# ronghanghu/vit_10b_fsdp_example

Measured on AMD Instinct MI355X. Metric: images/sec (whole node) for ViT-10B bs=128 224px --fake_data, higher is better.
Workload: dtype bf16; 1 GPU; model=ViT-10B (5120d/32h/32L, patch14, 224px), global_batch=128, seq_len=256, parallelism=fsdp1, grad_ckpt=True, grad_ckpt_blocks=13, fuse_residual=False, init=device

## Files before the change

__graft_entry__.py:

```python

import os
import subprocess
import sys


def build():
    env = dict(os.environ)
    env["PYTORCH_ROCM_ARCH"] = "gfx950"
    env.setdefault("MAX_JOBS", "8")
    repo = os.path.dirname(os.path.abspath(__file__))
    subprocess.check_call(
        [sys.executable, "setup.py", "build_ext", "--inplace"],
        cwd=repo, env=env,
    )
    import torch
    import vit_10b_fsdp_example_amd
    import vit_10b_fsdp_example_amd._C as _C

    required = [
        "layernorm_fwd", "layernorm_bwd", "layernorm_add_fwd",
        "fused_adamw", "multi_tensor_sqnorm", "cross_entropy_fwd",
        "fmha_fwd", "fmha_bwd", "fmha_fwd_qkv", "wgrad_gemm", "lt_gemm",
        "fwd_gemm", "fwd_gemm_gelu", "mfma32_probe",
    ]
    missing = [f for f in required if not hasattr(_C, f)]
    assert not missing, f"extension missing symbols: {missing}"
    print("build OK: vit_10b_fsdp_example_amd._C (gfx950)")


def smoke():
    import torch

    assert torch.cuda.is_available(), "smoke() needs a GPU"
    from vit_10b_fsdp_example_amd import dist as xdist
    from vit_10b_fsdp_example_amd.cli import parse_args
    from vit_10b_fsdp_example_amd.models import build_fsdp_vit_model
    from vit_10b_fsdp_example_amd.ops import (
        CrossEntropyLoss, FusedAdamW, has_ext,
    )

    assert has_ext(), "HIP extension _C not importable on the GPU box"
    device = xdist.init_distributed()
    cfg = parse_args([
        "--fake_data", "--image_size", "224", "--patch_size", "14",
        "--embed_dim", "640", "--num_heads", "4", "--num_blocks", "2",
        "--num_classes", "1000", "--batch_size", "8", "--num_workers", "0",
# ... 23 lines not shown
```

csrc/bindings.cpp:

```cpp

#include <torch/extension.h>

std::vector<torch::Tensor> layernorm_fwd(torch::Tensor x, torch::Tensor w,
                                         torch::Tensor b, double eps);
std::vector<torch::Tensor> layernorm_bwd(torch::Tensor dy, torch::Tensor x,
                                         torch::Tensor w, torch::Tensor mean,
                                         torch::Tensor rstd);
std::vector<torch::Tensor> layernorm_add_fwd(torch::Tensor x,
                                             torch::Tensor res,
                                             torch::Tensor w, torch::Tensor b,
                                             double eps);
std::vector<torch::Tensor> layernorm_add_bwd(torch::Tensor dy,
                                             torch::Tensor dsum,
                                             torch::Tensor sum,
                                             torch::Tensor w,
                                             torch::Tensor mean,
                                             torch::Tensor rstd);

void fused_adamw(std::vector<torch::Tensor> params,
                 std::vector<torch::Tensor> grads,
                 std::vector<torch::Tensor> exp_avgs,
                 std::vector<torch::Tensor> exp_avg_sqs,
                 std::vector<c10::optional<torch::Tensor>> mirrors,
                 double lr,
// ... 5 lines not shown
void multi_tensor_scale(std::vector<torch::Tensor> tensors, double factor);
void multi_tensor_scale_tensor(std::vector<torch::Tensor> tensors,
                               torch::Tensor factor);

std::vector<torch::Tensor> cross_entropy_fwd(torch::Tensor logits,
                                             torch::Tensor target);
torch::Tensor cross_entropy_bwd(torch::Tensor dloss, torch::Tensor logits,
                                torch::Tensor target, torch::Tensor lse);

std::vector<torch::Tensor> fmha_fwd(torch::Tensor q, torch::Tensor k,
                                    torch::Tensor v, double scale,
                                    double p_drop, long seed);
std::vector<torch::Tensor> fmha_bwd(torch::Tensor dout, torch::Tensor q,
                                    torch::Tensor k, torch::Tensor v,
                                    torch::Tensor o, torch::Tensor lse,
                                    double scale, double p_drop, long seed);
std::vector<torch::Tensor> fmha_fwd_qkv(torch::Tensor qkv, long num_heads,
                                        double scale, double p_drop,
                                        long seed);
torch::Tensor fmha_bwd_qkv(torch::Tensor dout, torch::Tensor qkv,
                           torch::Tensor o, torch::Tensor lse,
                           long num_heads, double scale, double p_drop,
                           long seed);
torch::Tensor mfma_probe(torch::Tensor a, torch::Tensor b);
torch::Tensor mfma32_probe(torch::Tensor a, torch::Tensor b);
torch::Tensor tr16_probe(long mode);
std::vector<torch::Tensor> wgrad_gemm(torch::Tensor a, torch::Tensor b,
                                      bool with_bias);
torch::Tensor fwd_gemm(torch::Tensor x, torch::Tensor w,
                       c10::optional<torch::Tensor> bias);
std::vector<torch::Tensor> fwd_gemm_gelu(torch::Tensor x, torch::Tensor w,
                                         torch::Tensor bias);
torch::Tensor lt_gemm(torch::Tensor a, torch::Tensor b, long algo_index,
                      c10::optional<torch::Tensor> bias);
std::vector<torch::Tensor> lt_gemm_gelu(torch::Tensor a, torch::Tensor b,
                                        c10::optional<torch::Tensor> bias,
                                        long algo_index);
std::vector<torch::Tensor> lt_gemm_dgelu_bgrad(torch::Tensor dy,
                                               torch::Tensor w,
                                               torch::Tensor aux,
                                               long algo_index);

PYBIND11_MODULE(TORCH_EXTENSION_NAME, m) {
  m.doc() = "MI355X-native CDNA4 kernels for the FSDP ViT framework";
  m.def("layernorm_fwd", &layernorm_fwd, "LayerNorm forward (bf16, fp32 stats)");
  m.def("layernorm_bwd", &layernorm_bwd, "LayerNorm backward");
// ... 17 lines not shown
  m.def("cross_entropy_fwd", &cross_entropy_fwd, "fused softmax CE forward");
  m.def("cross_entropy_bwd", &cross_entropy_bwd, "fused softmax CE backward");
  m.def("fmha_fwd", &fmha_fwd,
        "flash attention forward (bf16, head_dim<=192; in-kernel "
        "attention dropout via a counter-hash mask)",
        py::arg("q"), py::arg("k"), py::arg("v"), py::arg("scale"),
        py::arg("p_drop") = 0.0, py::arg("seed") = 0);
  m.def("fmha_bwd", &fmha_bwd,
        "flash attention backward (fused FA2-style; regenerates the "
        "dropout mask from the seed)",
        py::arg("dout"), py::arg("q"), py::arg("k"), py::arg("v"),
        py::arg("o"), py::arg("lse"), py::arg("scale"),
        py::arg("p_drop") = 0.0, py::arg("seed") = 0);
  m.def("fmha_fwd_qkv", &fmha_fwd_qkv,
        "flash attention forward on the fused [B,T,3,H,D] qkv projection "
        "(zero-copy strided IO, O returned as [B,T,E])",
        py::arg("qkv"), py::arg("num_heads"), py::arg("scale"),
        py::arg("p_drop") = 0.0, py::arg("seed") = 0);
  m.def("fmha_bwd_qkv", &fmha_bwd_qkv,
        "flash attention backward producing the fused dqkv [B,T,3,H,D]",
        py::arg("dout"), py::arg("qkv"), py::arg("o"), py::arg("lse"),
        py::arg("num_heads"), py::arg("scale"), py::arg("p_drop") = 0.0,
        py::arg("seed") = 0);
  m.def("mfma_probe", &mfma_probe, "16x16x32 bf16 MFMA layout probe");
  m.def("mfma32_probe", &mfma32_probe, "32x32x16 bf16 MFMA layout probe");
  m.def("tr16_probe", &tr16_probe, "ds_read_b64_tr_b16 semantics probe");
  m.def("wgrad_gemm", &wgrad_gemm,
        "C = A^T B weight-gradient GEMM (bf16, tr16 transpose reads)");
  m.def("fwd_gemm", &fwd_gemm,
        "C = X W^T forward Linear GEMM (+fused bias), hand-written CDNA4 "
        "MFMA (csrc/fgemm.hip)",
        py::arg("x"), py::arg("w"), py::arg("bias") = py::none());
  m.def("fwd_gemm_gelu", &fwd_gemm_gelu,
        "(gelu(X W^T + bias), pre-activation) with the EXACT erf GELU "
        "fused into the hand-written forward GEMM epilogue",
        py::arg("x"), py::arg("w"), py::arg("bias"));
  m.def("lt_gemm", &lt_gemm,
        "row-major bf16 GEMM (+optional fused bias epilogue) via "
        "hipblaslt-ext with an explicit algorithm index (-1 = library "
        "heuristic); offline-search apply path, see "
        "csrc/tools/hipblaslt_search.cpp",
        py::arg("a"), py::arg("b"), py::arg("algo_index") = -1,
        py::arg("bias") = py::none());
  m.def("lt_gemm_gelu", &lt_gemm_gelu,
        "(gelu(a@b+bias), pre-activation aux) in one hipblaslt-ext GEMM "
        "(GELU_AUX epilogue; tanh-approx GELU)",
// ... 9 lines not shown
```

csrc/fmha.hip:

```cpp

#ifndef VITFSDP_KERNELS_ONLY
#include <ATen/cuda/CUDAContext.h>
#include <torch/extension.h>

#include <cstdlib>
#include <cstring>
#include <type_traits>
#endif

#include "mfma_tiles.h"

namespace {

constexpr int kBlockThreads = 256;
constexpr int kKTile = 32;
constexpr int kMaxD = 192;

template <int D>
struct FmhaShapes {
  static constexpr int QSub = (D <= 96) ? 2 : 1;
  static constexpr int QTile = 64 * QSub;
  static constexpr int DP = ((D + 31) / 32) * 32;
  static constexpr int NKC = DP / 32;
  static constexpr int NC = D / 16;
// ... 488 lines not shown
        base0 + (unsigned)offsetof(typename S::SharedDKV, do_tile);
    mfma_tr_ring<NC, S::KStride>(pt_frag, do_lds_base, seg, col, dv_acc);
    mfma_tr_ring<NC, S::KStride>(dst_frag, q_lds_base, seg, col, dk_acc);
    if (has_next) {
      __syncthreads();
      write_qdo_tiles();
      __syncthreads();
    }
  }

#pragma unroll
  for (int r = 0; r < 4; ++r) {
    const int k_row = k_row0 + seg * 4 + r;
    if (k_row >= T) continue;
    const long out_base = qkv_off + (long)k_row * st.qt;
#pragma unroll
    for (int c = 0; c < NC; ++c) {
      dk[out_base + c * 16 + col] = (short)f32_to_bf16(dk_acc[c][r]);
      dv[out_base + c * 16 + col] = (short)f32_to_bf16(dv_acc[c][r]);
    }
  }
}

__global__ __launch_bounds__(64) void fmha_rowdot_kernel(
    const unsigned short* __restrict__ dout,
    const unsigned short* __restrict__ o, float* __restrict__ delta, int T,
    int H, int D, long sob, long soh, long sot) {
  const long row = blockIdx.x;
  const int t = (int)(row % T);
  const int h = (int)((row / T) % H);
  const long b = row / ((long)T * H);
  const long base = b * sob + (long)h * soh + (long)t * sot;
  float acc = 0.f;
  for (int i = threadIdx.x; i < D; i += 64)
    acc += bf16_to_f32(dout[base + i]) * bf16_to_f32(o[base + i]);
  acc = wave_all_sum(acc);
  if (threadIdx.x == 0) delta[row] = acc;
}

__global__ __launch_bounds__(256) void fmha_dsoftmax_kernel(
    const unsigned short* __restrict__ s_raw,
    const unsigned short* __restrict__ dp, const float* __restrict__ lse,
    const float* __restrict__ delta, unsigned short* __restrict__ p_out,
    unsigned short* __restrict__ ds_out, int T, float scale) {
  const long row = blockIdx.x;
  const float row_lse = lse[row];
  const float row_delta = delta[row];
// ... 146 lines not shown
  st.qb = (long)H * st.qh;
  st.qt = D;
  st.ob = st.qb;
  st.oh = st.qh;
  st.ot = st.qt;
  return st;
}

QkvStrides fused_qkv_strides(int T, int H, int D) {
  QkvStrides st;
  st.qt = 3L * H * D;
  st.qb = (long)T * st.qt;
  st.qh = D;
  st.ot = (long)H * D;
  st.ob = (long)T * st.ot;
  st.oh = D;
  return st;
}

torch::Tensor run_rowdot(const torch::Tensor& dout, const torch::Tensor& o,
                         int B, int H, int T, int D, const QkvStrides& st) {
  auto delta = torch::empty({B, H, T}, dout.options().dtype(torch::kFloat32));
  auto stream = at::cuda::getCurrentCUDAStream();
  hipLaunchKernelGGL(fmha_rowdot_kernel, dim3((long)B * H * T), dim3(64), 0,
                     stream, (const unsigned short*)dout.data_ptr(),
                     (const unsigned short*)o.data_ptr(),
                     delta.data_ptr<float>(), T, H, D, st.ob, st.oh, st.ot);
  HIP_CHECK_LAST();
  return delta;
}

}


std::vector<torch::Tensor> fmha_fwd(torch::Tensor q, torch::Tensor k,
                                    torch::Tensor v, double scale,
                                    double p_drop, long seed) {
  TORCH_CHECK(q.is_cuda() && q.is_contiguous() && k.is_contiguous() &&
              v.is_contiguous());
  TORCH_CHECK(q.scalar_type() == torch::kBFloat16, "fmha_fwd: bf16 only");
  TORCH_CHECK(q.dim() == 4, "fmha_fwd: [B, H, T, D]");
  const int B = q.size(0), H = q.size(1), T = q.size(2), D = q.size(3);
  TORCH_CHECK(D % 16 == 0 && D <= kMaxD,
              "fmha_fwd: head_dim must be a multiple of 16 and <= ", kMaxD);

  auto o = torch::empty_like(q);
  auto lse = torch::empty({B, H, T}, q.options().dtype(torch::kFloat32));
  FmhaArgs a{(const short*)q.data_ptr(), (const short*)k.data_ptr(),
             (const short*)v.data_ptr(), (short*)o.data_ptr(),
             B, H, T, contiguous_strides(H, T, D), (float)scale,
// ... 26 lines not shown
                       (const unsigned short*)dp.data_ptr(),
                       lse.data_ptr<float>(), delta.data_ptr<float>(),
                       (unsigned short*)p.data_ptr(),
                       (unsigned short*)ds.data_ptr(), T, (float)scale);
    HIP_CHECK_LAST();
    auto dv = at::matmul(p.transpose(-2, -1), dout);
    auto dq = at::matmul(ds, k);
    auto dk = at::matmul(ds.transpose(-2, -1), q);
    return {dq, dk, dv};
  }

  auto dq = torch::empty_like(q);
  auto dk = torch::empty_like(k);
  auto dv = torch::empty_like(v);
  FmhaArgs a{(const short*)q.data_ptr(), (const short*)k.data_ptr(),
             (const short*)v.data_ptr(), (short*)dout.data_ptr(),
             B, H, T, st, (float)scale, (float)p_drop, (unsigned)seed};
  VITFSDP_FMHA_DISPATCH(
      D, launch_fmha_bwd<kD>(a, lse, delta, (short*)dq.data_ptr(),
                             (short*)dk.data_ptr(), (short*)dv.data_ptr()));
  return {dq, dk, dv};
}


std::vector<torch::Tensor> fmha_fwd_qkv(torch::Tensor qkv, long num_heads,
                                        double scale, double p_drop,
                                        long seed) {
  TORCH_CHECK(qkv.is_cuda() && qkv.is_contiguous() && qkv.dim() == 5 &&
                  qkv.size(2) == 3 && qkv.size(3) == num_heads,
              "fmha_fwd_qkv: expected contiguous [B, T, 3, H, D]");
  TORCH_CHECK(qkv.scalar_type() == torch::kBFloat16, "fmha: bf16 only");
  const int B = qkv.size(0), T = qkv.size(1), H = qkv.size(3),
            D = qkv.size(4);
  TORCH_CHECK(D % 16 == 0 && D <= kMaxD,
              "fmha: head_dim must be a multiple of 16 and <= ", kMaxD);
  const QkvStrides st = fused_qkv_strides(T, H, D);

  auto o = torch::empty({B, T, (long)H * D}, qkv.options());
  auto lse = torch::empty({B, H, T}, qkv.options().dtype(torch::kFloat32));
  const short* base = (const short*)qkv.data_ptr();
  FmhaArgs a{base, base + (long)H * D, base + 2L * H * D,
             (short*)o.data_ptr(), B, H, T, st, (float)scale,
             (float)p_drop, (unsigned)seed};
  VITFSDP_FMHA_DISPATCH(D, launch_fmha_fwd<kD>(a, lse));
  return {o, lse};
}
// ... 24 lines not shown
```

csrc/layernorm.hip:

```cpp

#ifndef VITFSDP_KERNELS_ONLY
#include <ATen/cuda/CUDAContext.h>
#include <torch/extension.h>
#endif

#include "common.h"

namespace {

constexpr int kBlock = 256;
constexpr int kWaves = kBlock / WAVE_SIZE;

__global__ void ln_fwd_kernel(const ushort8_t* __restrict__ x,
                              const ushort8_t* __restrict__ w,
                              const ushort8_t* __restrict__ b,
                              ushort8_t* __restrict__ y,
                              float* __restrict__ mean_out,
                              float* __restrict__ rstd_out, int nvec,
                              float inv_d, float eps) {
  __shared__ float scratch[kWaves];
  const long row = blockIdx.x;
  const ushort8_t* xr = x + row * nvec;
  ushort8_t* yr = y + row * nvec;

// ... 69 lines not shown
  }
}

__global__ void ln_bwd_dwdb_partial_kernel(
    const unsigned short* __restrict__ dy, const unsigned short* __restrict__ x,
    const float* __restrict__ mean_in, const float* __restrict__ rstd_in,
    float* __restrict__ dw_part, float* __restrict__ db_part, int d,
    long n_rows, int rows_per_chunk) {
  const int col = blockIdx.x * kBlock + threadIdx.x;
  if (col >= d) return;
  const long row_begin = (long)blockIdx.y * rows_per_chunk;
  const long row_end = min(row_begin + rows_per_chunk, n_rows);
  float dw = 0.f, db = 0.f;
  for (long r = row_begin; r < row_end; ++r) {
    float dyv = bf16_to_f32(dy[r * d + col]);
    float xh = (bf16_to_f32(x[r * d + col]) - mean_in[r]) * rstd_in[r];
    dw += dyv * xh;
    db += dyv;
  }
  dw_part[(long)blockIdx.y * d + col] = dw;
  db_part[(long)blockIdx.y * d + col] = db;
}

__global__ void ln_bwd_dwdb_final_kernel(const float* __restrict__ dw_part,
                                         const float* __restrict__ db_part,
                                         unsigned short* __restrict__ dw,
                                         unsigned short* __restrict__ db,
                                         int d, int n_chunks) {
  const int col = blockIdx.x * kBlock + threadIdx.x;
  if (col >= d) return;
  float sw = 0.f, sb = 0.f;
  for (int c = 0; c < n_chunks; ++c) {
    sw += dw_part[(long)c * d + col];
    sb += db_part[(long)c * d + col];
  }
  dw[col] = f32_to_bf16(sw);
  db[col] = f32_to_bf16(sb);
}


__global__ void ln_add_fwd_kernel(const ushort8_t* __restrict__ x,
                                  const ushort8_t* __restrict__ res,
                                  const ushort8_t* __restrict__ w,
                                  const ushort8_t* __restrict__ b,
                                  ushort8_t* __restrict__ sum_out,
                                  ushort8_t* __restrict__ y,
                                  float* __restrict__ mean_out,
                                  float* __restrict__ rstd_out, int nvec,
                                  float inv_d, float eps) {
  __shared__ float scratch[kWaves];
  const long row = blockIdx.x;
  const ushort8_t* xr = x + row * nvec;
  const ushort8_t* rr = res + row * nvec;
  ushort8_t* sr = sum_out + row * nvec;
  ushort8_t* yr = y + row * nvec;

  float s = 0.f, ss = 0.f;
  for (int i = threadIdx.x; i < nvec; i += kBlock) {
    ushort8_t xv = xr[i], rv = rr[i], sv;
#pragma unroll
    for (int j = 0; j < 8; ++j) {
// ... 55 lines not shown
      sg += g;
      sgx += g * xh;
    }
  }
  sg = block_sum<kWaves>(sg, scratch) * inv_d;
  sgx = block_sum<kWaves>(sgx, scratch) * inv_d;

  for (int i = threadIdx.x; i < nvec; i += kBlock) {
    ushort8_t dv = dyr[i], sv = sr[i], wv = w[i], av = dsr[i], out;
#pragma unroll
    for (int j = 0; j < 8; ++j) {
      float g = bf16_to_f32(dv[j]) * bf16_to_f32(wv[j]);
      float xh = (bf16_to_f32(sv[j]) - mean) * rstd;
      out[j] = f32_to_bf16(rstd * (g - sg - xh * sgx) + bf16_to_f32(av[j]));
    }
    d1[i] = out;
    d2[i] = out;
  }
}

}

#ifndef VITFSDP_KERNELS_ONLY
std::vector<torch::Tensor> layernorm_fwd(torch::Tensor x, torch::Tensor w,
                                         torch::Tensor b, double eps) {
  TORCH_CHECK(x.is_cuda() && x.is_contiguous());
  TORCH_CHECK(x.scalar_type() == torch::kBFloat16, "layernorm_fwd: bf16 only");
  const int d = x.size(-1);
  TORCH_CHECK(d % 8 == 0, "layernorm_fwd: D must be a multiple of 8");
  const long n = x.numel() / d;
  auto y = torch::empty_like(x);
  auto opts = x.options().dtype(torch::kFloat32);
  auto mean = torch::empty({n}, opts);
  auto rstd = torch::empty({n}, opts);
  auto stream = at::cuda::getCurrentCUDAStream();
  hipLaunchKernelGGL(ln_fwd_kernel, dim3((unsigned)n), dim3(kBlock), 0, stream,
                     (const ushort8_t*)x.data_ptr(),
                     (const ushort8_t*)w.data_ptr(),
                     (const ushort8_t*)b.data_ptr(), (ushort8_t*)y.data_ptr(),
                     mean.data_ptr<float>(), rstd.data_ptr<float>(), d / 8,
                     1.f / d, (float)eps);
  HIP_CHECK_LAST();
  return {y, mean, rstd};
}

std::vector<torch::Tensor> layernorm_bwd(torch::Tensor dy, torch::Tensor x,
                                         torch::Tensor w, torch::Tensor mean,
                                         torch::Tensor rstd) {
  TORCH_CHECK(dy.is_cuda() && dy.is_contiguous() && x.is_contiguous());
  const int d = x.size(-1);
  const long n = x.numel() / d;
  auto dx = torch::empty_like(x);
  auto dw = torch::empty_like(w);
  auto db = torch::empty_like(w);
  auto stream = at::cuda::getCurrentCUDAStream();
  hipLaunchKernelGGL(ln_bwd_dx_kernel, dim3((unsigned)n), dim3(kBlock), 0,
                     stream, (const ushort8_t*)dy.data_ptr(),
                     (const ushort8_t*)x.data_ptr(),
                     (const ushort8_t*)w.data_ptr(), mean.data_ptr<float>(),
                     rstd.data_ptr<float>(), (ushort8_t*)dx.data_ptr(), d / 8,
                     1.f / d);
  HIP_CHECK_LAST();

  const int grid_x = (d + kBlock - 1) / kBlock;
  int n_chunks = std::max(1, 2048 / std::max(grid_x, 1));
  int rows_per_chunk = (int)((n + n_chunks - 1) / n_chunks);
  rows_per_chunk = std::max(rows_per_chunk, 16);
  n_chunks = (int)((n + rows_per_chunk - 1) / rows_per_chunk);
  auto opts = x.options().dtype(torch::kFloat32);
  auto dw_part = torch::empty({n_chunks, d}, opts);
  auto db_part = torch::empty({n_chunks, d}, opts);
  dim3 grid((d + kBlock - 1) / kBlock, n_chunks);
  hipLaunchKernelGGL(ln_bwd_dwdb_partial_kernel, grid, dim3(kBlock), 0, stream,
                     (const unsigned short*)dy.data_ptr(),
                     (const unsigned short*)x.data_ptr(),
                     mean.data_ptr<float>(), rstd.data_ptr<float>(),
                     dw_part.data_ptr<float>(), db_part.data_ptr<float>(), d, n,
                     rows_per_chunk);
  HIP_CHECK_LAST();
  hipLaunchKernelGGL(ln_bwd_dwdb_final_kernel, dim3((d + kBlock - 1) / kBlock),
                     dim3(kBlock), 0, stream, dw_part.data_ptr<float>(),
                     db_part.data_ptr<float>(),
                     (unsigned short*)dw.data_ptr(),
                     (unsigned short*)db.data_ptr(), d, n_chunks);
  HIP_CHECK_LAST();
  return {dx, dw, db};
}


std::vector<torch::Tensor> layernorm_add_fwd(torch::Tensor x,
                                             torch::Tensor res,
                                             torch::Tensor w, torch::Tensor b,
                                             double eps) {
  TORCH_CHECK(x.is_cuda() && x.is_contiguous() && res.is_contiguous());
  TORCH_CHECK(x.scalar_type() == torch::kBFloat16, "bf16 only");
  const int d = x.size(-1);
  TORCH_CHECK(d % 8 == 0, "layernorm_add_fwd: D must be a multiple of 8");
  const long n = x.numel() / d;
  auto sum = torch::empty_like(x);
  auto y = torch::empty_like(x);
  auto opts = x.options().dtype(torch::kFloat32);
  auto mean = torch::empty({n}, opts);
  auto rstd = torch::empty({n}, opts);
  auto stream = at::cuda::getCurrentCUDAStream();
  hipLaunchKernelGGL(ln_add_fwd_kernel, dim3((unsigned)n), dim3(kBlock), 0,
                     stream, (const ushort8_t*)x.data_ptr(),
                     (const ushort8_t*)res.data_ptr(),
                     (const ushort8_t*)w.data_ptr(),
                     (const ushort8_t*)b.data_ptr(),
                     (ushort8_t*)sum.data_ptr(), (ushort8_t*)y.data_ptr(),
                     mean.data_ptr<float>(), rstd.data_ptr<float>(), d / 8,
                     1.f / d, (float)eps);
  HIP_CHECK_LAST();
  return {sum, y, mean, rstd};
}

std::vector<torch::Tensor> layernorm_add_bwd(torch::Tensor dy,
                                             torch::Tensor dsum,
                                             torch::Tensor sum,
                                             torch::Tensor w,
                                             torch::Tensor mean,
                                             torch::Tensor rstd) {
  TORCH_CHECK(dy.is_cuda() && dy.is_contiguous() && dsum.is_contiguous() &&
              sum.is_contiguous());
  const int d = sum.size(-1);
  const long n = sum.numel() / d;
  auto dx1 = torch::empty_like(sum);
  auto dx2 = torch::empty_like(sum);
  auto stream = at::cuda::getCurrentCUDAStream();
  hipLaunchKernelGGL(ln_add_bwd_dx_kernel, dim3((unsigned)n), dim3(kBlock), 0,
                     stream, (const ushort8_t*)dy.data_ptr(),
                     (const ushort8_t*)dsum.data_ptr(),
                     (const ushort8_t*)sum.data_ptr(),
                     (const ushort8_t*)w.data_ptr(), mean.data_ptr<float>(),
                     rstd.data_ptr<float>(), (ushort8_t*)dx1.data_ptr(),
                     (ushort8_t*)dx2.data_ptr(), d / 8, 1.f / d);
  HIP_CHECK_LAST();

  auto dw = torch::empty_like(w);
  auto db = torch::empty_like(w);
  const int grid_x = (d + kBlock - 1) / kBlock;
  int n_chunks = std::max(1, 2048 / std::max(grid_x, 1));
  int rows_per_chunk = (int)((n + n_chunks - 1) / n_chunks);
  rows_per_chunk = std::max(rows_per_chunk, 16);
  n_chunks = (int)((n + rows_per_chunk - 1) / rows_per_chunk);
  auto opts = sum.options().dtype(torch::kFloat32);
  auto dw_part = torch::empty({n_chunks, d}, opts);
  auto db_part = torch::empty({n_chunks, d}, opts);
  dim3 grid(grid_x, n_chunks);
  hipLaunchKernelGGL(ln_bwd_dwdb_partial_kernel, grid, dim3(kBlock), 0, stream,
                     (const unsigned short*)dy.data_ptr(),
                     (const unsigned short*)sum.data_ptr(),
                     mean.data_ptr<float>(), rstd.data_ptr<float>(),
                     dw_part.data_ptr<float>(), db_part.data_ptr<float>(), d,
                     n, rows_per_chunk);
  HIP_CHECK_LAST();
  hipLaunchKernelGGL(ln_bwd_dwdb_final_kernel, dim3(grid_x), dim3(kBlock), 0,
                     stream, dw_part.data_ptr<float>(),
                     db_part.data_ptr<float>(), (unsigned short*)dw.data_ptr(),
                     (unsigned short*)db.data_ptr(), d, n_chunks);
  HIP_CHECK_LAST();
  return {dx1, dx2, dw, db};
}

#endif
```

setup.py:

```python

import os

from setuptools import setup

os.environ.setdefault("PYTORCH_ROCM_ARCH", "gfx950")

from torch.utils.cpp_extension import BuildExtension, CUDAExtension

ext = CUDAExtension(
    name="vit_10b_fsdp_example_amd._C",
    sources=[
        "csrc/bindings.cpp",
        "csrc/ltgemm.cpp",
        "csrc/layernorm.hip",
        "csrc/adamw.hip",
        "csrc/cross_entropy.hip",
        "csrc/fmha.hip",
        "csrc/wgemm.hip",
        "csrc/fgemm.hip",
        "csrc/probes.hip",
    ],
    libraries=["hipblaslt"],
    extra_compile_args={
        "cxx": ["-O3", "-std=c++17"],
        "nvcc": [
            "-O3",
            "-std=c++17",
            "--offload-arch=gfx950",
            "-Rpass-analysis=kernel-resource-usage",
        ],
    },
)

setup(
    name="vit_10b_fsdp_example_amd_ext",
    version="0.1.0",
    ext_modules=[ext],
    cmdclass={"build_ext": BuildExtension.with_options(use_ninja=True)},
)
```

vit_10b_fsdp_example_amd/ops/linear.py:

```python

import contextlib
import os

import torch
import torch.nn as nn
import torch.nn.functional as F
from torch.utils._python_dispatch import TorchDispatchMode

from ._extension import ext, use_hip
from ..tuning import lt_algo_table


_WGRAD_MODE = os.environ.get("VITFSDP_NATIVE_WGRAD", "0")
_NATIVE_WGRAD = _WGRAD_MODE == "1"
_NATIVE_WGRAD_DISPATCH = _WGRAD_MODE == "2"


def _use_native_wgrad(dy2, x2, w):
    if not _NATIVE_WGRAD:
        return False
    if not (dy2.is_cuda and dy2.dtype == torch.bfloat16):
        return False
    m, n = w.shape[0], w.shape[1]
    k = dy2.shape[0]
# ... 103 lines not shown



_GELU_CFG = {"d": 0, "hid": 0}

_FGEMM_MIN_TILES = int(os.environ.get("VITFSDP_FGEMM_MIN_TILES", "256"))


def configure_gelu_fusion(embed_dim, hidden_dim):
    if embed_dim != hidden_dim:
        _GELU_CFG["d"] = int(embed_dim)
        _GELU_CFG["hid"] = int(hidden_dim)


def _gelu_fusion_on():
    return (
        os.environ.get("VITFSDP_FUSED_GELU", "0") == "1"
        and _GELU_CFG["hid"] > 0
    )




class TunedGemmMode(TorchDispatchMode):

    def __init__(self, table=None, native_wgrad=None, handler=None):
        super().__init__()
        self.table = lt_algo_table() if table is None else table
        self.native_wgrad = (
            _NATIVE_WGRAD_DISPATCH if native_wgrad is None else native_wgrad
        )
        self._handler = handler
        self.hits = 0
        self.wgrad_hits = 0
        self.fused_gelu = _gelu_fusion_on()
        self._pending_gelu = {}
        self.gelu_hits = 0

    def _tuned_index(self, a, b):
        if not self.table:
            return None
        key = _dual_key(a, b)
        if key is None:
            return None
        return self.table.get(key)

    def _gpu_ok(self, t):
        if self._handler is not None:
            return True
        return t.is_cuda and t.dtype == torch.bfloat16 and use_hip(t)

    def _route(self, a, b, idx, bias=None):
        if self._handler is not None:
            return self._handler(a, b, idx, bias)
        return ext().lt_gemm(a, b, idx, bias)


    def _is_fc1_fwd(self, key):
        if not (
            key is not None
            and key[0] == "T" and key[1] == "N"
            and key[2] == _GELU_CFG["hid"] and key[4] == _GELU_CFG["d"]
        ):
            return False
        if self._handler is not None:
            return True
        hid, tok = key[2], key[3]
        return (
            tok % 256 == 0 and hid % 256 == 0 and key[4] % 64 == 0
            and (tok // 256) * (hid // 256) >= _FGEMM_MIN_TILES
        )

    def _fused_fc1_fwd(self, a, b, bias):
        if self._handler is not None:
            out, pre = self._handler(a, b, "gelu", bias)
        else:
            out, pre = ext().fwd_gemm_gelu(
                a.contiguous(), b.t().contiguous(), bias
            )
        self.gelu_hits += 1
        if len(self._pending_gelu) > 4:
            self._pending_gelu.clear()
        self._pending_gelu[pre.data_ptr()] = out
        return pre

    def __torch_dispatch__(self, func, types, args=(), kwargs=None):
        kwargs = kwargs or {}
        if func is torch.ops.aten.mm.default and self._gpu_ok(args[0]):
            a, b = args
            if (
                self.native_wgrad
                and self._handler is None
                and _is_wgrad_mm(a, b)
                and hasattr(ext(), "wgrad_gemm")
            ):
                self.wgrad_hits += 1
                (dw,) = ext().wgrad_gemm(a.t().contiguous(), b.contiguous(),
                                         False)
                return dw
            idx = self._tuned_index(a, b)
            if idx is not None:
                self.hits += 1
                return self._route(a, b, idx)
        elif (
            func is torch.ops.aten.addmm.default
            and len(args) == 3
            and kwargs.get("beta", 1) == 1
            and kwargs.get("alpha", 1) == 1
            and self._gpu_ok(args[1])
            and args[0].dim() == 1
        ):
            bias, a, b = args
            key = _dual_key(a, b)
            if (
                self.fused_gelu
                and self._is_fc1_fwd(key)
                and (self._handler is not None
                     or hasattr(ext(), "fwd_gemm_gelu"))
            ):
                return self._fused_fc1_fwd(a, b, bias)
            idx = self.table.get(key) if (self.table and key) else None
            if idx is not None:
                self.hits += 1
                return self._route(a, b, idx, bias)
        elif self.fused_gelu and func is torch.ops.aten.gelu.default:
            out = self._pending_gelu.pop(args[0].data_ptr(), None)
            if out is not None and out.shape == args[0].shape:
                return out
        return func(*args, **kwargs)


def gemm_dispatch_context():
    if lt_algo_table() or _gelu_fusion_on():
        return TunedGemmMode()
    if _NATIVE_WGRAD_DISPATCH:
        return NativeWgradMode()
    return contextlib.nullcontext()


def wgrad_backward_context():
    return gemm_dispatch_context()


class NativeLinear(nn.Linear):

    def forward(self, x):
        if _NATIVE_WGRAD:
            return _NativeLinearFn.apply(x, self.weight, self.bias)
        return F.linear(x, self.weight, self.bias)
```

Measured before the change: 65.66 images/sec.

## Fuse GELU backward with fc1 bias-grad colsum, fuse LayerNorm backward, vectorize rowdot

Adds a HIP kernel that computes the exact-erf GELU backward and the column sums of its output in one pass. A dispatch-mode hook intercepts aten.gelu_backward and then returns the stashed colsum for the following bias-gradient sum, so a separate reduction pass over the large MLP hidden activation is skipped. LayerNorm backward gains a fused single-kernel path for dx and dw/db partials, and its final reduction is parallelised across row chunks. The attention Delta rowdot kernel is vectorised to 8-lane 16-byte loads with several rows per block. The costs are more complex dispatch-interception logic that relies on tensor storage identity, and bf16 colsum precision.

```diff
diff --git a/__graft_entry__.py b/__graft_entry__.py
--- a/__graft_entry__.py
+++ b/__graft_entry__.py
@@ -21,7 +21,8 @@
         "layernorm_fwd", "layernorm_bwd", "layernorm_add_fwd",
         "fused_adamw", "multi_tensor_sqnorm", "cross_entropy_fwd",
         "fmha_fwd", "fmha_bwd", "fmha_fwd_qkv", "wgrad_gemm", "lt_gemm",
-        "fwd_gemm", "fwd_gemm_gelu", "mfma32_probe",
+        "fwd_gemm", "fwd_gemm_gelu", "mfma32_probe", "fmha_rowdot",
+        "gelu_bwd_colsum",
     ]
     missing = [f for f in required if not hasattr(_C, f)]
     assert not missing, f"extension missing symbols: {missing}"
diff --git a/csrc/bindings.cpp b/csrc/bindings.cpp
--- a/csrc/bindings.cpp
+++ b/csrc/bindings.cpp
@@ -51,6 +51,8 @@
                            torch::Tensor o, torch::Tensor lse,
                            long num_heads, double scale, double p_drop,
                            long seed);
+torch::Tensor fmha_rowdot(torch::Tensor dout, torch::Tensor o);
+std::vector<torch::Tensor> gelu_bwd_colsum(torch::Tensor dy, torch::Tensor x);
 torch::Tensor mfma_probe(torch::Tensor a, torch::Tensor b);
 torch::Tensor mfma32_probe(torch::Tensor a, torch::Tensor b);
 torch::Tensor tr16_probe(long mode);
@@ -114,6 +116,14 @@
         py::arg("dout"), py::arg("qkv"), py::arg("o"), py::arg("lse"),
         py::arg("num_heads"), py::arg("scale"), py::arg("p_drop") = 0.0,
         py::arg("seed") = 0);
+  m.def("fmha_rowdot", &fmha_rowdot,
+        "Delta = rowsum(dO * O) of the attention backward, fp32 [B,H,T], "
+        "for contiguous [B,H,T,D] operands",
+        py::arg("dout"), py::arg("o"));
+  m.def("gelu_bwd_colsum", &gelu_bwd_colsum,
+        "(dx, colsum): exact-erf GELU backward and the bf16 column sums "
+        "of dx over all rows (fc1 bias gradient) in one pass",
+        py::arg("dy"), py::arg("x"));
   m.def("mfma_probe", &mfma_probe, "16x16x32 bf16 MFMA layout probe");
   m.def("mfma32_probe", &mfma32_probe, "32x32x16 bf16 MFMA layout probe");
   m.def("tr16_probe", &tr16_probe, "ds_read_b64_tr_b16 semantics probe");
diff --git a/csrc/fmha.hip b/csrc/fmha.hip
--- a/csrc/fmha.hip
+++ b/csrc/fmha.hip
@@ -534,7 +534,68 @@
   }
 }
 
-__global__ __launch_bounds__(64) void fmha_rowdot_kernel(
+constexpr int kRowdotLanes = 8;
+constexpr int kRowdotRows = kBlockThreads / kRowdotLanes;
+constexpr int kRowdotMaxLoads = kMaxD / 8 / kRowdotLanes;
+
+__global__ __launch_bounds__(kBlockThreads) void fmha_rowdot_kernel(
+    const ushort8_t* __restrict__ dout, const ushort8_t* __restrict__ o,
+    float* __restrict__ delta, int n_rows, int T, int H, int nvec,
+    long sob, long soh, long sot ,
+    int h_fast) {
+  const int g = threadIdx.x % kRowdotLanes;
+  const int slot = threadIdx.x / kRowdotLanes;
+  for (long r0 = (long)blockIdx.x * kRowdotRows; r0 < n_rows;
+       r0 += (long)gridDim.x * kRowdotRows) {
+    const bool ok = r0 + slot < n_rows;
+    const unsigned r = ok ? (unsigned)(r0 + slot) : 0u;
+    unsigned b, h, t;
+    if (h_fast) {
+      h = r % (unsigned)H;
+      t = (r / (unsigned)H) % (unsigned)T;
+    } else {
+      t = r % (unsigned)T;
+      h = (r / (unsigned)T) % (unsigned)H;
+    }
+    b = r / ((unsigned)T * (unsigned)H);
+    const long base = (long)b * sob + (long)h * soh + (long)t * sot;
+
+    ushort8_t dv[kRowdotMaxLoads], ov[kRowdotMaxLoads];
+#pragma unroll
+    for (int k = 0; k < kRowdotMaxLoads; ++k) {
+      const int v = g + k * kRowdotLanes;
+      if (ok && v < nvec) {
+        dv[k] = dout[base + v];
+        ov[k] = o[base + v];
+      }
+    }
+    float acc[8];
+#pragma unroll
+    for (int j = 0; j < 8; ++j) acc[j] = 0.f;
+#pragma unroll
+    for (int k = 0; k < kRowdotMaxLoads; ++k) {
+      const int v = g + k * kRowdotLanes;
+      if (ok && v < nvec) {
+#pragma unroll
+        for (int j = 0; j < 8; ++j)
+          acc[j] += bf16_to_f32(dv[k][j]) * bf16_to_f32(ov[k][j]);
+      }
+    }
+#pragma unroll
+    for (int off = kRowdotLanes / 2; off > 0; off >>= 1) {
+#pragma unroll
+      for (int j = 0; j < 8; ++j) acc[j] += __shfl_xor(acc[j], off);
+    }
+#pragma unroll
+    for (int j = 0; j < 4; ++j) acc[j] += acc[j + 4];
+    acc[0] += acc[2];
+    acc[1] += acc[3];
+    acc[0] += acc[1];
+    if (ok && g == 0) delta[((long)b * H + h) * T + t] = acc[0];
+  }
+}
+
+__global__ __launch_bounds__(64) void fmha_rowdot_scalar_kernel(
     const unsigned short* __restrict__ dout,
     const unsigned short* __restrict__ o, float* __restrict__ delta, int T,
     int H, int D, long sob, long soh, long sot) {
@@ -727,10 +788,28 @@
                          int B, int H, int T, int D, const QkvStrides& st) {
   auto delta = torch::empty({B, H, T}, dout.options().dtype(torch::kFloat32));
   auto stream = at::cuda::getCurrentCUDAStream();
-  hipLaunchKernelGGL(fmha_rowdot_kernel, dim3((long)B * H * T), dim3(64), 0,
-                     stream, (const unsigned short*)dout.data_ptr(),
-                     (const unsigned short*)o.data_ptr(),
-                     delta.data_ptr<float>(), T, H, D, st.ob, st.oh, st.ot);
+  const long n_rows = (long)B * H * T;
+  if (n_rows == 0) return delta;
+  const bool aligned =
+      ((reinterpret_cast<uintptr_t>(dout.data_ptr()) |
+        reinterpret_cast<uintptr_t>(o.data_ptr())) & 15) == 0 &&
+      D % 8 == 0 && D <= kMaxD && st.ob % 8 == 0 && st.oh % 8 == 0 &&
+      st.ot % 8 == 0;
+  if (aligned && n_rows < (1L << 31)) {
+    const long n_blocks =
+        std::min<long>((n_rows + kRowdotRows - 1) / kRowdotRows, 2048);
+    hipLaunchKernelGGL(fmha_rowdot_kernel, dim3((unsigned)n_blocks),
+                       dim3(kBlockThreads), 0, stream,
+                       (const ushort8_t*)dout.data_ptr(),
+                       (const ushort8_t*)o.data_ptr(), delta.data_ptr<float>(),
+                       (int)n_rows, T, H, D / 8, st.ob / 8, st.oh / 8,
+                       st.ot / 8, st.oh < st.ot ? 1 : 0);
+  } else {
+    hipLaunchKernelGGL(fmha_rowdot_scalar_kernel, dim3(n_rows), dim3(64), 0,
+                       stream, (const unsigned short*)dout.data_ptr(),
+                       (const unsigned short*)o.data_ptr(),
+                       delta.data_ptr<float>(), T, H, D, st.ob, st.oh, st.ot);
+  }
   HIP_CHECK_LAST();
   return delta;
 }
@@ -803,6 +882,22 @@
   return {dq, dk, dv};
 }
 
+torch::Tensor fmha_rowdot(torch::Tensor dout, torch::Tensor o) {
+  TORCH_CHECK(dout.is_cuda() && o.is_cuda() && dout.is_contiguous() &&
+                  o.is_contiguous(),
+              "fmha_rowdot: contiguous GPU tensors");
+  TORCH_CHECK(dout.scalar_type() == torch::kBFloat16 &&
+                  o.scalar_type() == torch::kBFloat16,
+              "fmha_rowdot: bf16 only");
+  TORCH_CHECK(dout.dim() == 4 && dout.sizes() == o.sizes(),
+              "fmha_rowdot: two [B, H, T, D] tensors of one shape");
+  const int B = dout.size(0), H = dout.size(1), T = dout.size(2),
+            D = dout.size(3);
+  TORCH_CHECK(D % 16 == 0 && D <= kMaxD,
+              "fmha_rowdot: head_dim must be a multiple of 16 and <= ", kMaxD);
+  return run_rowdot(dout, o, B, H, T, D, contiguous_strides(H, T, D));
+}
+
 
 std::vector<torch::Tensor> fmha_fwd_qkv(torch::Tensor qkv, long num_heads,
                                         double scale, double p_drop,
diff --git a/csrc/gelu.hip b/csrc/gelu.hip
--- /dev/null
+++ b/csrc/gelu.hip
@@ -0,0 +1,119 @@
+
+#ifndef VITFSDP_KERNELS_ONLY
+#include <ATen/cuda/CUDAContext.h>
+#include <torch/extension.h>
+#endif
+
+#include "common.h"
+
+namespace {
+
+constexpr int kBlock = 256;
+
+__device__ __forceinline__ float gelu_bwd_one(float dy, float x) {
+  constexpr float kAlpha = 0.70710678118654752440f;
+  constexpr float kBeta = 0.39894228040143267794f;
+  const float cdf = 0.5f * (1.f + erff(x * kAlpha));
+  const float pdf = expf(-0.5f * x * x) * kBeta;
+  return dy * (cdf + x * pdf);
+}
+
+__global__ __launch_bounds__(kBlock) void gelu_bwd_colsum_kernel(
+    const ushort8_t* __restrict__ dy, const ushort8_t* __restrict__ x,
+    ushort8_t* __restrict__ dx, float* __restrict__ part, int nvec,
+    long n_rows, int rows_per_chunk) {
+  const int vc = blockIdx.x * kBlock + threadIdx.x;
+  if (vc >= nvec) return;
+  const long row_begin = (long)blockIdx.y * rows_per_chunk;
+  const long row_end = min(row_begin + rows_per_chunk, n_rows);
+  float acc[8];
+#pragma unroll
+  for (int j = 0; j < 8; ++j) acc[j] = 0.f;
+#pragma unroll 4
+  for (long r = row_begin; r < row_end; ++r) {
+    const long i = r * nvec + vc;
+    const ushort8_t dv = dy[i], xv = x[i];
+    ushort8_t out;
+#pragma unroll
+    for (int j = 0; j < 8; ++j) {
+      out[j] = f32_to_bf16(gelu_bwd_one(bf16_to_f32(dv[j]), bf16_to_f32(xv[j])));
+      acc[j] += bf16_to_f32(out[j]);
+    }
+    dx[i] = out;
+  }
+  float4* p = reinterpret_cast<float4*>(part + ((long)blockIdx.y * nvec + vc) * 8);
+  p[0] = make_float4(acc[0], acc[1], acc[2], acc[3]);
+  p[1] = make_float4(acc[4], acc[5], acc[6], acc[7]);
+}
+
+constexpr int kFinalCols = 32;
+constexpr int kFinalSlices = kBlock / kFinalCols;
+
+__global__ __launch_bounds__(kBlock) void gelu_colsum_final_kernel(
+    const float* __restrict__ part, unsigned short* __restrict__ out, int hid,
+    int n_chunks) {
+  __shared__ float s_s[kFinalSlices][kFinalCols];
+  const int c = threadIdx.x % kFinalCols;
+  const int slice = threadIdx.x / kFinalCols;
+  const int col = blockIdx.x * kFinalCols + c;
+  float s = 0.f;
+  if (col < hid) {
+#pragma unroll 4
+    for (int ch = slice; ch < n_chunks; ch += kFinalSlices)
+      s += part[(long)ch * hid + col];
+  }
+  s_s[slice][c] = s;
+  __syncthreads();
+  if (slice == 0 && col < hid) {
+#pragma unroll
+    for (int k = 1; k < kFinalSlices; ++k) s += s_s[k][c];
+    out[col] = f32_to_bf16(s);
+  }
+}
+
+}
+
+#ifndef VITFSDP_KERNELS_ONLY
+std::vector<torch::Tensor> gelu_bwd_colsum(torch::Tensor dy, torch::Tensor x) {
+  TORCH_CHECK(dy.is_cuda() && x.is_cuda() && dy.is_contiguous() &&
+                  x.is_contiguous(),
+              "gelu_bwd_colsum: contiguous GPU tensors");
+  TORCH_CHECK(dy.scalar_type() == torch::kBFloat16 &&
+                  x.scalar_type() == torch::kBFloat16,
+              "gelu_bwd_colsum: bf16 only");
+  TORCH_CHECK(dy.dim() >= 1 && dy.sizes() == x.sizes(),
+              "gelu_bwd_colsum: dy and x must have one shape");
+  const long hid = dy.size(-1);
+  TORCH_CHECK(hid > 0 && hid % 8 == 0,
+              "gelu_bwd_colsum: last dim must be a multiple of 8, got ", hid);
+  TORCH_CHECK(hid < (1L << 31), "gelu_bwd_colsum: last dim too large");
+  const long n = dy.numel() / hid;
+  auto dx = torch::empty_like(dy);
+  auto colsum = torch::empty({hid}, dy.options());
+  if (n == 0) {
+    colsum.zero_();
+    return {dx, colsum};
+  }
+  const int nvec = (int)(hid / 8);
+  const int grid_x = (nvec + kBlock - 1) / kBlock;
+  long n_chunks = std::max(1, 2048 / grid_x);
+  long rows_per_chunk = std::max<long>((n + n_chunks - 1) / n_chunks, 16);
+  n_chunks = (n + rows_per_chunk - 1) / rows_per_chunk;
+  TORCH_CHECK(n_chunks <= 65535, "gelu_bwd_colsum: too many rows");
+  auto part = torch::empty({n_chunks, hid},
+                           dy.options().dtype(torch::kFloat32));
+  auto stream = at::cuda::getCurrentCUDAStream();
+  hipLaunchKernelGGL(gelu_bwd_colsum_kernel, dim3(grid_x, (unsigned)n_chunks),
+                     dim3(kBlock), 0, stream, (const ushort8_t*)dy.data_ptr(),
+                     (const ushort8_t*)x.data_ptr(), (ushort8_t*)dx.data_ptr(),
+                     part.data_ptr<float>(), nvec, n, (int)rows_per_chunk);
+  HIP_CHECK_LAST();
+  hipLaunchKernelGGL(gelu_colsum_final_kernel,
+                     dim3((unsigned)((hid + kFinalCols - 1) / kFinalCols)),
+                     dim3(kBlock), 0, stream, part.data_ptr<float>(),
+                     (unsigned short*)colsum.data_ptr(), (int)hid,
+                     (int)n_chunks);
+  HIP_CHECK_LAST();
+  return {dx, colsum};
+}
+#endif
diff --git a/csrc/layernorm.hip b/csrc/layernorm.hip
--- a/csrc/layernorm.hip
+++ b/csrc/layernorm.hip
@@ -115,21 +115,149 @@
   db_part[(long)blockIdx.y * d + col] = db;
 }
 
+constexpr int kFinalCols = 32;
+constexpr int kFinalSlices = kBlock / kFinalCols;
+
 __global__ void ln_bwd_dwdb_final_kernel(const float* __restrict__ dw_part,
                                          const float* __restrict__ db_part,
                                          unsigned short* __restrict__ dw,
                                          unsigned short* __restrict__ db,
                                          int d, int n_chunks) {
-  const int col = blockIdx.x * kBlock + threadIdx.x;
-  if (col >= d) return;
+  __shared__ float sw_s[kFinalSlices][kFinalCols];
+  __shared__ float sb_s[kFinalSlices][kFinalCols];
+  const int c = threadIdx.x % kFinalCols;
+  const int slice = threadIdx.x / kFinalCols;
+  const int col = blockIdx.x * kFinalCols + c;
   float sw = 0.f, sb = 0.f;
-  for (int c = 0; c < n_chunks; ++c) {
-    sw += dw_part[(long)c * d + col];
-    sb += db_part[(long)c * d + col];
-  }
-  dw[col] = f32_to_bf16(sw);
-  db[col] = f32_to_bf16(sb);
-}
+  if (col < d) {
+#pragma unroll 4
+    for (int ch = slice; ch < n_chunks; ch += kFinalSlices) {
+      sw += dw_part[(long)ch * d + col];
+      sb += db_part[(long)ch * d + col];
+    }
+  }
+  sw_s[slice][c] = sw;
+  sb_s[slice][c] = sb;
+  __syncthreads();
+  if (slice == 0 && col < d) {
+#pragma unroll
+    for (int s = 1; s < kFinalSlices; ++s) {
+      sw += sw_s[s][c];
+      sb += sb_s[s][c];
+    }
+    dw[col] = f32_to_bf16(sw);
+    db[col] = f32_to_bf16(sb);
+  }
+}
+
+constexpr int kFusedBlocks = 768;
+constexpr int kMaxVpt = 4;
+
+template <int VPT, bool ADD>
+__global__ __launch_bounds__(kBlock) void ln_bwd_fused_kernel(
+    const ushort8_t* __restrict__ dy, const ushort8_t* __restrict__ dsum,
+    const ushort8_t* __restrict__ x, const ushort8_t* __restrict__ w,
+    const float* __restrict__ mean_in, const float* __restrict__ rstd_in,
+    ushort8_t* __restrict__ dx1, ushort8_t* __restrict__ dx2,
+    float* __restrict__ dw_part, float* __restrict__ db_part, int nvec,
+    long n_rows, float inv_d) {
+  __shared__ float scratch[kWaves];
+  float dw_acc[VPT][8], db_acc[VPT][8];
+  ushort8_t wv[VPT];
+#pragma unroll
+  for (int k = 0; k < VPT; ++k) {
+    const int i = threadIdx.x + k * kBlock;
+    if (i < nvec) wv[k] = w[i];
+#pragma unroll
+    for (int j = 0; j < 8; ++j) {
+      dw_acc[k][j] = 0.f;
+      db_acc[k][j] = 0.f;
+    }
+  }
+
+  for (long row = blockIdx.x; row < n_rows; row += gridDim.x) {
+    const ushort8_t* dyr = dy + row * nvec;
+    const ushort8_t* xr = x + row * nvec;
+    const float mean = mean_in[row];
+    const float rstd = rstd_in[row];
+
+    float sg = 0.f, sgx = 0.f;
+#pragma unroll
+    for (int k = 0; k < VPT; ++k) {
+      const int i = threadIdx.x + k * kBlock;
+      if (i < nvec) {
+        const ushort8_t dv = dyr[i], xv = xr[i];
+#pragma unroll
+        for (int j = 0; j < 8; ++j) {
+          float g = bf16_to_f32(dv[j]) * bf16_to_f32(wv[k][j]);
+          float xh = (bf16_to_f32(xv[j]) - mean) * rstd;
+          sg += g;
+          sgx += g * xh;
+        }
+      }
+    }
+    sg = block_sum<kWaves>(sg, scratch) * inv_d;
+    sgx = block_sum<kWaves>(sgx, scratch) * inv_d;
+
+#pragma unroll
+    for (int k = 0; k < VPT; ++k) {
+      const int i = threadIdx.x + k * kBlock;
+      if (i < nvec) {
+        const ushort8_t dv = dyr[i], xv = xr[i];
+        ushort8_t av, out;
+        if (ADD) av = dsum[row * nvec + i];
+#pragma unroll
+        for (int j = 0; j < 8; ++j) {
+          float dyf = bf16_to_f32(dv[j]);
+          float g = dyf * bf16_to_f32(wv[k][j]);
+          float xh = (bf16_to_f32(xv[j]) - mean) * rstd;
+          if (ADD) {
+            out[j] = f32_to_bf16(rstd * (g - sg - xh * sgx) +
+                                 bf16_to_f32(av[j]));
+          } else {
+            out[j] = f32_to_bf16(rstd * (g - sg - xh * sgx));
+          }
+          dw_acc[k][j] += dyf * xh;
+          db_acc[k][j] += dyf;
+        }
+        dx1[row * nvec + i] = out;
+        if (ADD) dx2[row * nvec + i] = out;
+      }
+    }
+  }
+
+  const long part_row = (long)blockIdx.x * nvec * 8;
+#pragma unroll
+  for (int k = 0; k < VPT; ++k) {
+    const int i = threadIdx.x + k * kBlock;
+    if (i < nvec) {
+      float4* pw = reinterpret_cast<float4*>(dw_part + part_row + (long)i * 8);
+      float4* pb = reinterpret_cast<float4*>(db_part + part_row + (long)i * 8);
+      pw[0] = make_float4(dw_acc[k][0], dw_acc[k][1], dw_acc[k][2],
+                          dw_acc[k][3]);
+      pw[1] = make_float4(dw_acc[k][4], dw_acc[k][5], dw_acc[k][6],
+                          dw_acc[k][7]);
+      pb[0] = make_float4(db_acc[k][0], db_acc[k][1], db_acc[k][2],
+                          db_acc[k][3]);
+      pb[1] = make_float4(db_acc[k][4], db_acc[k][5], db_acc[k][6],
+                          db_acc[k][7]);
+    }
+  }
+}
+
+#ifdef VITFSDP_KERNELS_ONLY
+#define VITFSDP_INSTANTIATE_LN(VPT_, ADD_)                                   \
+  template __global__ void ln_bwd_fused_kernel<VPT_, ADD_>(                  \
+      const ushort8_t*, const ushort8_t*, const ushort8_t*,                  \
+      const ushort8_t*, const float*, const float*, ushort8_t*, ushort8_t*,  \
+      float*, float*, int, long, float);
+VITFSDP_INSTANTIATE_LN(1, false)
+VITFSDP_INSTANTIATE_LN(3, false)
+VITFSDP_INSTANTIATE_LN(3, true)
+VITFSDP_INSTANTIATE_LN(4, false)
+VITFSDP_INSTANTIATE_LN(4, true)
+#undef VITFSDP_INSTANTIATE_LN
+#endif
 
 
 __global__ void ln_add_fwd_kernel(const ushort8_t* __restrict__ x,
@@ -231,6 +359,84 @@
 }
 
 #ifndef VITFSDP_KERNELS_ONLY
+namespace {
+
+void launch_dwdb_final(const torch::Tensor& dw_part,
+                       const torch::Tensor& db_part, torch::Tensor& dw,
+                       torch::Tensor& db, int d, int n_chunks,
+                       hipStream_t stream) {
+  hipLaunchKernelGGL(ln_bwd_dwdb_final_kernel,
+                     dim3((d + kFinalCols - 1) / kFinalCols), dim3(kBlock), 0,
+                     stream, dw_part.data_ptr<float>(),
+                     db_part.data_ptr<float>(),
+                     (unsigned short*)dw.data_ptr(),
+                     (unsigned short*)db.data_ptr(), d, n_chunks);
+  HIP_CHECK_LAST();
+}
+
+void dwdb_two_stage(const torch::Tensor& dy, const torch::Tensor& x,
+                    const torch::Tensor& mean, const torch::Tensor& rstd,
+                    torch::Tensor& dw, torch::Tensor& db, int d, long n,
+                    hipStream_t stream) {
+  const int grid_x = (d + kBlock - 1) / kBlock;
+  int n_chunks = std::max(1, 2048 / std::max(grid_x, 1));
+  int rows_per_chunk = (int)((n + n_chunks - 1) / n_chunks);
+  rows_per_chunk = std::max(rows_per_chunk, 16);
+  n_chunks = (int)((n + rows_per_chunk - 1) / rows_per_chunk);
+  auto opts = x.options().dtype(torch::kFloat32);
+  auto dw_part = torch::empty({n_chunks, d}, opts);
+  auto db_part = torch::empty({n_chunks, d}, opts);
+  hipLaunchKernelGGL(ln_bwd_dwdb_partial_kernel, dim3(grid_x, n_chunks),
+                     dim3(kBlock), 0, stream,
+                     (const unsigned short*)dy.data_ptr(),
+                     (const unsigned short*)x.data_ptr(),
+                     mean.data_ptr<float>(), rstd.data_ptr<float>(),
+                     dw_part.data_ptr<float>(), db_part.data_ptr<float>(), d, n,
+                     rows_per_chunk);
+  HIP_CHECK_LAST();
+  launch_dwdb_final(dw_part, db_part, dw, db, d, n_chunks, stream);
+}
+
+template <bool ADD>
+void launch_bwd_fused(const torch::Tensor& dy, const torch::Tensor* dsum,
+                      const torch::Tensor& x, const torch::Tensor& w,
+                      const torch::Tensor& mean, const torch::Tensor& rstd,
+                      torch::Tensor& dx1, torch::Tensor* dx2,
+                      torch::Tensor& dw, torch::Tensor& db, int d, long n,
+                      hipStream_t stream) {
+  const int nvec = d / 8;
+  const int n_blocks = (int)std::min<long>(n, kFusedBlocks);
+  auto opts = x.options().dtype(torch::kFloat32);
+  auto dw_part = torch::empty({n_blocks, d}, opts);
+  auto db_part = torch::empty({n_blocks, d}, opts);
+  auto launch = [&](auto vpt) {
+    hipLaunchKernelGGL(
+        (ln_bwd_fused_kernel<decltype(vpt)::value, ADD>), dim3(n_blocks),
+        dim3(kBlock), 0, stream, (const ushort8_t*)dy.data_ptr(),
+        ADD ? (const ushort8_t*)dsum->data_ptr() : nullptr,
+        (const ushort8_t*)x.data_ptr(), (const ushort8_t*)w.data_ptr(),
+        mean.data_ptr<float>(), rstd.data_ptr<float>(),
+        (ushort8_t*)dx1.data_ptr(),
+        ADD ? (ushort8_t*)dx2->data_ptr() : nullptr,
+        dw_part.data_ptr<float>(), db_part.data_ptr<float>(), nvec, n,
+        1.f / d);
+  };
+  switch ((nvec + kBlock - 1) / kBlock) {
+    case 1: launch(std::integral_constant<int, 1>{}); break;
+    case 2: launch(std::integral_constant<int, 2>{}); break;
+    case 3: launch(std::integral_constant<int, 3>{}); break;
+    default: launch(std::integral_constant<int, 4>{}); break;
+  }
+  HIP_CHECK_LAST();
+  launch_dwdb_final(dw_part, db_part, dw, db, d, n_blocks, stream);
+}
+
+inline bool fused_bwd_fits(int d) {
+  return d % 8 == 0 && d / 8 <= kMaxVpt * kBlock;
+}
+
+}
+
 std::vector<torch::Tensor> layernorm_fwd(torch::Tensor x, torch::Tensor w,
                                          torch::Tensor b, double eps) {
   TORCH_CHECK(x.is_cuda() && x.is_contiguous());
@@ -263,6 +469,16 @@
   auto dw = torch::empty_like(w);
   auto db = torch::empty_like(w);
   auto stream = at::cuda::getCurrentCUDAStream();
+  if (n == 0) {
+    dw.zero_();
+    db.zero_();
+    return {dx, dw, db};
+  }
+  if (fused_bwd_fits(d)) {
+    launch_bwd_fused<false>(dy, nullptr, x, w, mean, rstd, dx, nullptr, dw, db,
+                            d, n, stream);
+    return {dx, dw, db};
+  }
   hipLaunchKernelGGL(ln_bwd_dx_kernel, dim3((unsigned)n), dim3(kBlock), 0,
                      stream, (const ushort8_t*)dy.data_ptr(),
                      (const ushort8_t*)x.data_ptr(),
@@ -270,29 +486,7 @@
                      rstd.data_ptr<float>(), (ushort8_t*)dx.data_ptr(), d / 8,
                      1.f / d);
   HIP_CHECK_LAST();
-
-  const int grid_x = (d + kBlock - 1) / kBlock;
-  int n_chunks = std::max(1, 2048 / std::max(grid_x, 1));
-  int rows_per_chunk = (int)((n + n_chunks - 1) / n_chunks);
-  rows_per_chunk = std::max(rows_per_chunk, 16);
-  n_chunks = (int)((n + rows_per_chunk - 1) / rows_per_chunk);
-  auto opts = x.options().dtype(torch::kFloat32);
-  auto dw_part = torch::empty({n_chunks, d}, opts);
-  auto db_part = torch::empty({n_chunks, d}, opts);
-  dim3 grid((d + kBlock - 1) / kBlock, n_chunks);
-  hipLaunchKernelGGL(ln_bwd_dwdb_partial_kernel, grid, dim3(kBlock), 0, stream,
-                     (const unsigned short*)dy.data_ptr(),
-                     (const unsigned short*)x.data_ptr(),
-                     mean.data_ptr<float>(), rstd.data_ptr<float>(),
-                     dw_part.data_ptr<float>(), db_part.data_ptr<float>(), d, n,
-                     rows_per_chunk);
-  HIP_CHECK_LAST();
-  hipLaunchKernelGGL(ln_bwd_dwdb_final_kernel, dim3((d + kBlock - 1) / kBlock),
-                     dim3(kBlock), 0, stream, dw_part.data_ptr<float>(),
-                     db_part.data_ptr<float>(),
-                     (unsigned short*)dw.data_ptr(),
-                     (unsigned short*)db.data_ptr(), d, n_chunks);
-  HIP_CHECK_LAST();
+  dwdb_two_stage(dy, x, mean, rstd, dw, db, d, n, stream);
   return {dx, dw, db};
 }
 
@@ -336,7 +530,19 @@
   const long n = sum.numel() / d;
   auto dx1 = torch::empty_like(sum);
   auto dx2 = torch::empty_like(sum);
+  auto dw = torch::empty_like(w);
+  auto db = torch::empty_like(w);
   auto stream = at::cuda::getCurrentCUDAStream();
+  if (n == 0) {
+    dw.zero_();
+    db.zero_();
+    return {dx1, dx2, dw, db};
+  }
+  if (fused_bwd_fits(d)) {
+    launch_bwd_fused<true>(dy, &dsum, sum, w, mean, rstd, dx1, &dx2, dw, db, d,
+                           n, stream);
+    return {dx1, dx2, dw, db};
+  }
   hipLaunchKernelGGL(ln_add_bwd_dx_kernel, dim3((unsigned)n), dim3(kBlock), 0,
                      stream, (const ushort8_t*)dy.data_ptr(),
                      (const ushort8_t*)dsum.data_ptr(),
@@ -345,30 +551,7 @@
                      rstd.data_ptr<float>(), (ushort8_t*)dx1.data_ptr(),
                      (ushort8_t*)dx2.data_ptr(), d / 8, 1.f / d);
   HIP_CHECK_LAST();
-
-  auto dw = torch::empty_like(w);
-  auto db = torch::empty_like(w);
-  const int grid_x = (d + kBlock - 1) / kBlock;
-  int n_chunks = std::max(1, 2048 / std::max(grid_x, 1));
-  int rows_per_chunk = (int)((n + n_chunks - 1) / n_chunks);
-  rows_per_chunk = std::max(rows_per_chunk, 16);
-  n_chunks = (int)((n + rows_per_chunk - 1) / rows_per_chunk);
-  auto opts = sum.options().dtype(torch::kFloat32);
-  auto dw_part = torch::empty({n_chunks, d}, opts);
-  auto db_part = torch::empty({n_chunks, d}, opts);
-  dim3 grid(grid_x, n_chunks);
-  hipLaunchKernelGGL(ln_bwd_dwdb_partial_kernel, grid, dim3(kBlock), 0, stream,
-                     (const unsigned short*)dy.data_ptr(),
-                     (const unsigned short*)sum.data_ptr(),
-                     mean.data_ptr<float>(), rstd.data_ptr<float>(),
-                     dw_part.data_ptr<float>(), db_part.data_ptr<float>(), d,
-                     n, rows_per_chunk);
-  HIP_CHECK_LAST();
-  hipLaunchKernelGGL(ln_bwd_dwdb_final_kernel, dim3(grid_x), dim3(kBlock), 0,
-                     stream, dw_part.data_ptr<float>(),
-                     db_part.data_ptr<float>(), (unsigned short*)dw.data_ptr(),
-                     (unsigned short*)db.data_ptr(), d, n_chunks);
-  HIP_CHECK_LAST();
+  dwdb_two_stage(dy, sum, mean, rstd, dw, db, d, n, stream);
   return {dx1, dx2, dw, db};
 }
 
diff --git a/setup.py b/setup.py
--- a/setup.py
+++ b/setup.py
@@ -16,6 +16,7 @@
         "csrc/adamw.hip",
         "csrc/cross_entropy.hip",
         "csrc/fmha.hip",
+        "csrc/gelu.hip",
         "csrc/wgemm.hip",
         "csrc/fgemm.hip",
         "csrc/probes.hip",
diff --git a/vit_10b_fsdp_example_amd/ops/linear.py b/vit_10b_fsdp_example_amd/ops/linear.py
--- a/vit_10b_fsdp_example_amd/ops/linear.py
+++ b/vit_10b_fsdp_example_amd/ops/linear.py
@@ -149,9 +149,18 @@
 
 
 
+def _dgelu_dbias_on():
+    return (
+        os.environ.get("VITFSDP_FUSED_DGELU_DBIAS", "1") != "0"
+        and _GELU_CFG["hid"] > 0
+    )
+
+
+
 class TunedGemmMode(TorchDispatchMode):
 
-    def __init__(self, table=None, native_wgrad=None, handler=None):
+    def __init__(self, table=None, native_wgrad=None, handler=None,
+                 dgelu_handler=None):
         super().__init__()
         self.table = lt_algo_table() if table is None else table
         self.native_wgrad = (
@@ -163,6 +172,17 @@
         self.fused_gelu = _gelu_fusion_on()
         self._pending_gelu = {}
         self.gelu_hits = 0
+        self._dgelu_handler = dgelu_handler
+        self.fused_dgelu = _dgelu_dbias_on() and (
+            dgelu_handler is not None or self._handler is None
+        )
+        self._dgelu_stash = None
+        self.dgelu_hits = 0
+        self.dbias_hits = 0
+
+    def __exit__(self, exc_type, exc_val, exc_tb):
+        self._dgelu_stash = None
+        return super().__exit__(exc_type, exc_val, exc_tb)
 
     def _tuned_index(self, a, b):
         if not self.table:
@@ -208,8 +228,66 @@
         self.gelu_hits += 1
         if len(self._pending_gelu) > 4:
             self._pending_gelu.clear()
-        self._pending_gelu[pre.data_ptr()] = out
+        self._pending_gelu[pre.data_ptr()] = (pre, out)
         return pre
+
+
+    def _is_mlp_dgelu(self, args, kwargs):
+        if len(args) != 2 or kwargs.get("approximate", "none") != "none":
+            return False
+        dy, x = args
+        if not (
+            dy.dim() >= 2
+            and dy.shape[-1] == _GELU_CFG["hid"]
+            and dy.shape == x.shape
+            and dy.is_contiguous() and x.is_contiguous()
+        ):
+            return False
+        if self._dgelu_handler is not None:
+            return True
+        return (
+            dy.is_cuda and dy.dtype == torch.bfloat16
+            and x.dtype == torch.bfloat16
+            and dy.shape[-1] % 8 == 0
+            and use_hip(dy)
+        )
+
+    def _fused_dgelu(self, dy, x):
+        if self._dgelu_handler is not None:
+            dx, colsum = self._dgelu_handler(dy, x)
+        else:
+            dx, colsum = ext().gelu_bwd_colsum(dy, x)
+        self.dgelu_hits += 1
+        self._dgelu_stash = (dx, colsum)
+        return dx
+
+    def _stashed_dbias(self, args, kwargs):
+        if self._dgelu_stash is None or kwargs.get("dtype") is not None:
+            return None
+        dx, colsum = self._dgelu_stash
+        t = args[0]
+        dims = args[1] if len(args) > 1 else None
+        keepdim = args[2] if len(args) > 2 else kwargs.get("keepdim", False)
+        if not (
+            isinstance(t, torch.Tensor)
+            and dims is not None
+            and t.dtype == dx.dtype
+            and t.device == dx.device
+            and t.untyped_storage().data_ptr()
+            == dx.untyped_storage().data_ptr()
+            and t.storage_offset() == dx.storage_offset()
+            and t.numel() == dx.numel()
+            and t.dim() >= 2
+            and t.shape[-1] == dx.shape[-1]
+            and t.is_contiguous()
+            and sorted(d % t.dim() for d in dims) == list(range(t.dim() - 1))
+        ):
+            return None
+        self._dgelu_stash = None
+        self.dbias_hits += 1
+        if keepdim:
+            return colsum.view([1] * (t.dim() - 1) + [t.shape[-1]])
+        return colsum
 
     def __torch_dispatch__(self, func, types, args=(), kwargs=None):
         kwargs = kwargs or {}
@@ -251,14 +329,24 @@
                 self.hits += 1
                 return self._route(a, b, idx, bias)
         elif self.fused_gelu and func is torch.ops.aten.gelu.default:
-            out = self._pending_gelu.pop(args[0].data_ptr(), None)
+            _, out = self._pending_gelu.pop(args[0].data_ptr(), (None, None))
             if out is not None and out.shape == args[0].shape:
                 return out
+        elif self.fused_dgelu and func is torch.ops.aten.gelu_backward.default:
+            if self._is_mlp_dgelu(args, kwargs):
+                return self._fused_dgelu(*args)
+        elif (
+            self._dgelu_stash is not None
+            and func is torch.ops.aten.sum.dim_IntList
+        ):
+            out = self._stashed_dbias(args, kwargs)
+            if out is not None:
+                return out
         return func(*args, **kwargs)
 
 
 def gemm_dispatch_context():
-    if lt_algo_table() or _gelu_fusion_on():
+    if lt_algo_table() or _gelu_fusion_on() or _dgelu_dbias_on():
         return TunedGemmMode()
     if _NATIVE_WGRAD_DISPATCH:
         return NativeWgradMode()
```

Result: faster. 66.37 images/sec, median of 6 (+1.1%).
